# SYSTRAN/faster-whisper

Hardware: AMD Instinct MI355X
Metric: audio-sec/sec (RTF) large-v3 fp16 beam=5 batch=16 (higher is better)
Workload: dtype f16

## Files before the change

### faster_whisper_amd/_lib.py

```python
import ctypes as C
import os

import numpy as np

_HERE = os.path.dirname(os.path.abspath(__file__))
LIB_PATH = os.environ.get("FWAMD_LIB") or os.path.join(_HERE, "libfwamd.so")

FW_OK = 0
FW_EINVAL = -1
FW_ENODEV = -2
FW_ENOMEM = -3
FW_ERUNTIME = -4
FW_ENOSPC = -5

COMPUTE_FLOAT16 = 0
COMPUTE_INT8_FLOAT16 = 1
FW_DT_F32 = 0
FW_DT_F16 = 1
FW_MAX_ALIGN_HEADS = 64


class FwConfig(C.Structure):
    _fields_ = [
        ("n_mels", C.c_int32), ("n_audio_ctx", C.c_int32), ("d_model", C.c_int32), ("n_heads", C.c_int32),
        ("n_enc_layers", C.c_int32), ("n_dec_layers", C.c_int32), ("n_vocab", C.c_int32),
        ("n_text_ctx", C.c_int32), ("is_multilingual", C.c_int32),
        ("tok_eot", C.c_int32), ("tok_sot", C.c_int32), ("tok_lang_begin", C.c_int32), ("n_langs", C.c_int32),
        ("tok_translate", C.c_int32), ("tok_transcribe", C.c_int32), ("tok_sot_lm", C.c_int32),
        ("tok_sot_prev", C.c_int32), ("tok_no_speech", C.c_int32), ("tok_no_timestamps", C.c_int32),
        ("tok_timestamp_begin", C.c_int32),
        ("n_suppress_begin", C.c_int32), ("suppress_begin", C.c_int32 * 8),
        ("n_align_heads", C.c_int32), ("align_heads", C.c_int32 * (2 * FW_MAX_ALIGN_HEADS)),
    ]


class FwWeight(C.Structure):
    _fields_ = [("name", C.c_char_p), ("data", C.c_void_p), ("dtype", C.c_int32), ("ndim", C.c_int32),
                ("dims", C.c_int64 * 4)]


class FwGenOpts(C.Structure):
    _fields_ = [
        ("beam_size", C.c_int32), ("patience", C.c_float), ("num_hypotheses", C.c_int32),
        ("length_penalty", C.c_float), ("repetition_penalty", C.c_float), ("no_repeat_ngram_size", C.c_int32),
        ("max_length", C.c_int32), ("return_scores", C.c_int32), ("return_no_speech_prob", C.c_int32),
        ("max_initial_timestamp_index", C.c_int32), ("suppress_blank", C.c_int32),
        ("suppress_tokens", C.POINTER(C.c_int32)), ("n_suppress_tokens", C.c_int32),
        ("sampling_topk", C.c_int32), ("sampling_temperature", C.c_float), ("seed", C.c_uint64),
        ("min_new_tokens", C.c_int32),
    ]


class FwVadWeights(C.Structure):
    _fields_ = [
        ("stft_basis", C.c_void_p), ("conv_w", C.c_void_p * 4), ("conv_b", C.c_void_p * 4),
        ("lstm_w", C.c_void_p), ("lstm_r", C.c_void_p), ("lstm_b", C.c_void_p), ("dec_w", C.c_void_p),
        ("dec_b", C.c_float),
    ]


SYMBOLS = [
    "fw_last_error", "fw_abi_version", "fw_device_count",
    "fw_model_create", "fw_model_free", "fw_model_info", "fw_model_blob", "fw_model_create_from_blob_dev",
    "fw_model_set_decode_batch", "fw_model_decode_batch", "fw_model_join_decoder", "fw_model_decode_stats",
    "fw_model_set_merge_wait", "fw_model_set_decode_lanes", "fw_model_run_capacity", "fw_dec_big_min_rows", "fw_dec_big_min_rows_of", "fw_test_knob",
    "fw_test_idle_lead_chunks",
    "fw_pack_blob_size", "fw_pack_blob_copy", "fw_pack_blob_free",
    "fw_logmel", "fw_logmel_full",
    "fw_encode", "fw_encode_pcm", "fw_encode_pcm_dev", "fw_tensor_shape", "fw_tensor_to_host",
    "fw_tensor_from_host", "fw_tensor_free",
    "fw_generate", "fw_generate_lp", "fw_detect_language", "fw_align",
    "fw_prof_enable", "fw_prof_reset", "fw_prof_count", "fw_prof_name", "fw_prof_get", "fw_synchronize",
    "fw_dev_alloc", "fw_dev_free", "fw_dev_upload",
    "fw_test_gemm", "fw_test_layernorm", "fw_test_attention", "fw_test_dec_linear", "fw_test_dec_logits", "fw_test_logits_rules",
    "fw_test_dec_self_attn", "fw_test_dec_cross_attn", "fw_test_dec_cross_probs", "fw_test_dec_softmax_pick", "fw_bench_gemm", "fw_bench_dec_linear", "fw_bench_attention",
    "fw_bench_gemm_epi", "fw_bench_dec_linear_epi",
    "fw_test_gemm_ex", "fw_test_cross_kv_frag_index", "fw_test_quant_rows", "fw_test_layernorm_frag",
    "fw_test_dec_beam_update", "fw_test_dec_embed", "fw_test_align_post",
    "fw_test_logits_rules_lp", "fw_test_dec_beam_update_lp",
    "fw_test_logits_rules_smp_tab", "fw_test_graph_captures",
    "fw_vad_create", "fw_vad_forward", "fw_vad_free", "fw_vad_forward_dev", "fw_vad_forward_audio_dev",
    "fw_vad_forward_audio_batch_dev",
    "fw_flac_info", "fw_flac_decode",
    "fw_resample_filter", "fw_resample_dev", "fw_bench_resample",
]

_lib = None


class FwError(RuntimeError):
    pass


def load():
    global _lib
    if _lib is not None:
        return _lib
    if not os.path.exists(LIB_PATH):
        raise FwError(
            f"{LIB_PATH} not found: build it with `python -c 'import __graft_entry__ as g; g.build()'` "
            "(hipcc --offload-arch=gfx950). faster_whisper_amd has no CPU fallback.")
    lib = C.CDLL(LIB_PATH)
    vp, i32, i64, f32p = C.c_void_p, C.c_int32, C.c_int64, C.POINTER(C.c_float)
    i32p, i64p = C.POINTER(C.c_int32), C.POINTER(C.c_int64)
    lib.fw_last_error.restype = C.c_char_p
    lib.fw_abi_version.restype = i32
    lib.fw_device_count.restype = i32
    lib.fw_model_create.argtypes = [C.POINTER(FwConfig), C.POINTER(FwWeight), i32, i32, i32, i32, i32, C.POINTER(vp)]
    lib.fw_model_free.argtypes = [vp]
    lib.fw_model_free.restype = None
    lib.fw_model_info.argtypes = [vp, C.POINTER(FwConfig), i32p, i32p, i32p, i32p]
    lib.fw_model_blob.argtypes = [vp, C.POINTER(vp), i64p]
    lib.fw_model_create_from_blob_dev.argtypes = [C.POINTER(FwConfig), vp, i64, i32, i32, i32, i32, C.POINTER(vp)]
    lib.fw_model_set_decode_batch.argtypes = [vp, i32]
    lib.fw_model_decode_batch.argtypes = [vp]
    lib.fw_model_decode_batch.restype = i32
    lib.fw_model_run_capacity.argtypes = [vp]
    lib.fw_model_run_capacity.restype = i32
    lib.fw_dec_big_min_rows.restype = i32
    if hasattr(lib, "fw_dec_big_min_rows_of"):
        lib.fw_dec_big_min_rows_of.restype = i32
        lib.fw_dec_big_min_rows_of.argtypes = [i32, i32]
    if hasattr(lib, "fw_flac_info"):
        lib.fw_flac_info.argtypes = [vp, i64, i32p, i32p, i32p, i64p]
        lib.fw_flac_decode.argtypes = [vp, i64, vp, i64, i64p, i32p]
    if hasattr(lib, "fw_test_knob"):
        lib.fw_test_knob.argtypes = [i32, i32]
    if hasattr(lib, "fw_test_idle_lead_chunks"):
        lib.fw_test_idle_lead_chunks.argtypes = [i64, i32, i32, i64, i32]
        lib.fw_test_idle_lead_chunks.restype = i64
    lib.fw_model_join_decoder.argtypes = [vp, vp]
    lib.fw_model_set_merge_wait.argtypes = [vp, i32, i32]
    lib.fw_model_set_decode_lanes.argtypes = [vp, i32]
    lib.fw_model_decode_stats.argtypes = [vp, i64p, i64p, i64p, i32p]
    lib.fw_pack_blob_size.argtypes = [C.POINTER(FwConfig), C.POINTER(FwWeight), i32, i32, i64p, C.POINTER(vp)]
    lib.fw_pack_blob_copy.argtypes = [vp, vp, i64]
    lib.fw_pack_blob_free.argtypes = [vp]
    lib.fw_pack_blob_free.restype = None
    lib.fw_logmel.argtypes = [vp, vp, i64p, i32, vp, i32p]
    lib.fw_logmel_full.argtypes = [vp, vp, i64, vp, i64]
    lib.fw_encode.argtypes = [vp, vp, i32, C.POINTER(vp)]
    lib.fw_encode_pcm.argtypes = [vp, vp, i64p, i32, C.POINTER(vp)]
    lib.fw_encode_pcm_dev.argtypes = [vp, vp, i64p, i32, C.POINTER(vp)]
    lib.fw_tensor_shape.argtypes = [vp, i32p, i32p, i32p]
    lib.fw_tensor_to_host.argtypes = [vp, vp, vp]
    lib.fw_tensor_from_host.argtypes = [vp, vp, i32, C.POINTER(vp)]
    lib.fw_tensor_free.argtypes = [vp]
    lib.fw_tensor_free.restype = None
    lib.fw_generate.argtypes = [vp, vp, i32p, i32p, i32, C.POINTER(FwGenOpts), i32p, i32p, f32p, f32p]
    if hasattr(lib, "fw_generate_lp"):
        lib.fw_generate_lp.argtypes = [vp, vp, i32p, i32p, i32, C.POINTER(FwGenOpts), i32p, i32p, f32p, f32p, f32p, f32p]
    lib.fw_detect_language.argtypes = [vp, vp, i32, i32p, f32p]
    lib.fw_align.argtypes = [vp, vp, i32p, i32, i32p, i32p, i32p, i32, i32, i32, i32p, i32p, f32p]
    lib.fw_prof_enable.argtypes = [vp, i32]
    lib.fw_prof_enable.restype = None
    lib.fw_prof_reset.argtypes = [vp]
    lib.fw_prof_reset.restype = None
    lib.fw_prof_count.restype = i32
    lib.fw_prof_name.argtypes = [i32]
    lib.fw_prof_name.restype = C.c_char_p
    lib.fw_prof_get.argtypes = [vp, i32, C.POINTER(C.c_double), i64p, C.POINTER(C.c_double), C.POINTER(C.c_double)]
    lib.fw_synchronize.argtypes = [vp]
    lib.fw_dev_alloc.argtypes = [vp, i64, C.POINTER(vp)]
    lib.fw_dev_free.argtypes = [vp, vp]
    lib.fw_dev_upload.argtypes = [vp, vp, vp, i64]
    lib.fw_test_gemm.argtypes = [vp, vp, vp, vp, vp, i32, i32, i32, i32, i32, vp]
    lib.fw_test_dec_linear.argtypes = [vp, vp, vp, vp, vp, vp, vp, i32, i32, i32, i32, i32, vp, vp]
    lib.fw_test_dec_logits.argtypes = [vp, vp, i32, vp]
    lib.fw_test_logits_rules.argtypes = [vp, vp, i32, vp, i32, vp, C.POINTER(FwGenOpts), i32, vp, vp]
    if hasattr(lib, "fw_test_dec_self_attn"):
        lib.fw_test_dec_self_attn.argtypes = [vp, vp, vp, vp, vp, i32, i32, i32, i32, i32, i32, i32, i32, i32, i32, i32, vp]
        lib.fw_test_dec_cross_attn.argtypes = [vp, vp, vp, vp, i32, i32, i32, i32, i32, i32, vp, vp, i32, C.c_float, vp]
        lib.fw_test_dec_cross_probs.argtypes = [vp, vp, vp, i32, i32, i32, vp, i32, i32, i32, i32, vp]
        lib.fw_test_dec_softmax_pick.argtypes = [vp, vp, i32, i32, i32, vp, i32, vp]
    lib.fw_bench_attention.argtypes = [vp, i32, i32, i32, i32, i32, f32p]
    lib.fw_bench_gemm.argtypes = [vp, i32, i32, i32, i32, i32, i32, i32, i32, f32p]
    lib.fw_bench_dec_linear.argtypes = [vp, i32, i32, i32, i32, i32, i32, f32p]
    if hasattr(lib, "fw_bench_gemm_epi"):
        lib.fw_bench_gemm_epi.argtypes = [vp, i32, i32, i32, i32, i32, i32, i32, i32, i32, i32, i32, f32p]
        lib.fw_bench_dec_linear_epi.argtypes = [vp, i32, i32, i32, i32, i32, i32, i32, i32, i32, f32p]
    lib.fw_test_layernorm.argtypes = [vp, vp, vp, vp, i32, i32, vp]
    lib.fw_test_attention.argtypes = [vp, vp, vp, vp, i32, i32, i32, vp]
    if hasattr(lib, "fw_test_gemm_ex"):
        lib.fw_test_gemm_ex.argtypes = [vp, vp, i64, i64, i64, vp, vp, vp, i64, i64, i64, vp, i64, i64, i64, i64, i64,
                                        i32, i32, i32, i32, i32, i32, i32, i32, i32, vp, vp]
        lib.fw_test_cross_kv_frag_index.argtypes = [i32, i32, i32, vp]
        lib.fw_test_quant_rows.argtypes = [vp, vp, i32, i32, i64, vp, vp, i32, vp, vp]
        lib.fw_test_layernorm_frag.argtypes = [vp, vp, vp, vp, i32, i32, i32, vp]
    if hasattr(lib, "fw_test_dec_beam_update"):
        f32 = C.c_float
        lib.fw_test_dec_beam_update.argtypes = [vp, i32, i32, i32, i32, i32, i32, i32, i32, f32, i32, vp, vp, vp, vp, vp,
                                                i32, f32, vp, vp, vp, vp, vp, vp, vp, vp, vp, vp, vp]
        lib.fw_test_dec_embed.argtypes = [vp, vp, i32, vp, i32, vp, i32, i32, i32, i32, i32, i32, f32, vp, vp]
        lib.fw_test_align_post.argtypes = [vp, vp, i32, i32, i32, i32, vp, vp, i32, vp]
    if hasattr(lib, "fw_test_dec_beam_update_lp"):
        f32 = C.c_float
        lib.fw_test_logits_rules_lp.argtypes = [vp, vp, i32, vp, i32, vp, C.POINTER(FwGenOpts), i32, vp, vp, vp]
        lib.fw_test_dec_beam_update_lp.argtypes = [vp, i32, i32, i32, i32, i32, i32, i32, i32, f32, i32, vp, vp, vp, vp, vp,
                                                   vp, vp, i32, f32, vp, vp, vp, vp, vp, vp, vp, vp, vp, vp, vp, vp, vp]
    if hasattr(lib, "fw_test_graph_captures"):
        lib.fw_test_logits_rules_smp_tab.argtypes = [vp, vp, i32, vp, i32, vp, C.POINTER(FwGenOpts), i32, vp, vp, vp, vp, vp, vp]
        lib.fw_test_graph_captures.argtypes = [vp, i64p]
    lib.fw_vad_create.argtypes = [C.POINTER(FwVadWeights), C.POINTER(vp)]
    lib.fw_vad_forward.argtypes = [vp, vp, i64, i32, vp, vp, vp]
    lib.fw_vad_free.argtypes = [vp]
    lib.fw_vad_forward_dev.argtypes = [vp, i32, vp, i64, vp, vp, vp]
    if hasattr(lib, "fw_vad_forward_audio_dev"):
        lib.fw_vad_forward_audio_dev.argtypes = [vp, i32, vp, i64, vp, vp, vp]
    if hasattr(lib, "fw_vad_forward_audio_batch_dev"):
        lib.fw_vad_forward_audio_batch_dev.argtypes = [vp, i32, vp, vp, i32, vp, vp, vp]
    lib.fw_vad_free.restype = None
    if hasattr(lib, "fw_resample_dev"):
        f64 = C.c_double
        lib.fw_resample_filter.argtypes = [i32, i32, i32, f64, vp, i64p, i32p, i32p]
        lib.fw_resample_dev.argtypes = [i32, vp, i64, i32, i32, i32, f64, i32, vp, i64]
        lib.fw_bench_resample.argtypes = [i32, vp, i64, i32, i32, i32, f64, i32, i32, f32p]
    _lib = lib
    return lib


def check(rc: int):
    if rc == FW_OK:
        return
    msg = load().fw_last_error().decode("utf-8", "replace")
    if rc in (FW_EINVAL, FW_ENOSPC):
        raise ValueError(msg)
    raise RuntimeError(f"libfwamd error {rc}: {msg}")


def ptr(a: np.ndarray):
    return a.ctypes.data_as(C.c_void_p)


def as_i32p(a: np.ndarray):
    return a.ctypes.data_as(C.POINTER(C.c_int32))


def as_i64p(a: np.ndarray):
    return a.ctypes.data_as(C.POINTER(C.c_int64))


def as_f32p(a: np.ndarray):
    return a.ctypes.data_as(C.POINTER(C.c_float))
```

### faster_whisper_amd/csrc/attn_enc.hip

```cpp
#include "common.h"
#include "kernels.h"

#define AE_Q 128
#define AE_KV 64
#define AE_VSTRIDE 68
#define AE_LAG 5.0f

__global__ __launch_bounds__(256) void attn_enc_kernel(const half_t* __restrict__ q, const half_t* __restrict__ k,
                                                       int64_t ld, int64_t qk_bstride,
                                                       const half_t* __restrict__ vt, int64_t ldvt,
                                                       int64_t vt_bstride, half_t* __restrict__ out, int64_t ldo,
                                                       int64_t o_bstride, int T, int H, int n_pairs, int n_qt,
                                                       int order) {
  __shared__ __attribute__((aligned(16))) half_t sK[2][AE_KV * 64];
  __shared__ __attribute__((aligned(16))) half_t sV[2][64 * AE_VSTRIDE];

  const int tid = threadIdx.x, lane = tid & 63, wave = tid >> 6;
  const int hi = lane >> 5, l31 = lane & 31;
  const int xcd = blockIdx.x & 7, idx = blockIdx.x >> 3;
  const int pair = order ? (int)blockIdx.x / n_qt : (idx / n_qt) * 8 + xcd;
  if (pair >= n_pairs) return;
  const int b = pair / H, h = pair - b * H, q0 = (order ? (int)blockIdx.x % n_qt : idx % n_qt) * AE_Q;

  const half_t* qb = q + (size_t)b * qk_bstride + h * 64;
  const half_t* kb = k + (size_t)b * qk_bstride + h * 64;
  const half_t* vb = vt + (size_t)b * vt_bstride + (size_t)(h * 64) * ldvt;

  half8_t qf[4];
  {
    int qr = q0 + wave * 32 + l31;
    if (qr > T - 1) qr = T - 1;
    const half_t* qp = qb + (size_t)qr * ld + hi * 8;
#pragma unroll
    for (int ks = 0; ks < 4; ++ks) {
      half8_t v = *reinterpret_cast<const half8_t*>(qp + ks * 16);
#pragma unroll
      for (int e = 0; e < 8; ++e) v[e] = (half_t)((float)v[e] * (0.125f * 1.4426950408889634f));
      qf[ks] = v;
    }
  }

  const int c = tid & 7, r0 = tid >> 3;
  const int nkt = (T + AE_KV - 1) / AE_KV;
  intx4 rk[2], rv[2];
  auto gload = [&](int kt) {
#pragma unroll
    for (int i = 0; i < 2; ++i) {
      const int row = r0 + 32 * i;
      int key = kt * AE_KV + row;
      if (key > T - 1) key = T - 1;
      rk[i] = *reinterpret_cast<const intx4*>(kb + (size_t)key * ld + c * 8);
      rv[i] = *reinterpret_cast<const intx4*>(vb + (size_t)row * ldvt + kt * AE_KV + c * 8);
    }
  };
  auto lstore = [&](int buf) {
#pragma unroll
    for (int i = 0; i < 2; ++i) {
      const int row = r0 + 32 * i;
      *reinterpret_cast<intx4*>(&sK[buf][row * 64 + ((c ^ ((row >> 1) & 7)) << 3)]) = rk[i];
      intx2* dv = reinterpret_cast<intx2*>(&sV[buf][row * AE_VSTRIDE + c * 8]);
      dv[0] = intx2{rv[i][0], rv[i][1]};
      dv[1] = intx2{rv[i][2], rv[i][3]};
    }
  };

  gload(0);
  lstore(0);
  __syncthreads();

  floatx16 o[2] = {floatx16{0}, floatx16{0}};
  floatx16 lsum = floatx16{0};
  const half8_t ones8 = {(half_t)1.f, (half_t)1.f, (half_t)1.f, (half_t)1.f, (half_t)1.f, (half_t)1.f, (half_t)1.f, (half_t)1.f};
  float m_ref = 0.f;
  floatx16 cneg = floatx16{0};

  for (int kt = 0; kt < nkt; ++kt) {
    const int cur = kt & 1;
    const bool more = (kt + 1) < nkt;
    if (more) gload(kt + 1);

    floatx16 s[2];
#pragma unroll
    for (int ks = 0; ks < 4; ++ks) {
      const int chunk = ks * 2 + hi;
#pragma unroll
      for (int kb2 = 0; kb2 < 2; ++kb2) {
        const int row = kb2 * 32 + l31;
        const half8_t kf = *reinterpret_cast<const half8_t*>(&sK[cur][row * 64 + ((chunk ^ ((row >> 1) & 7)) << 3)]);
        s[kb2] = __builtin_amdgcn_mfma_f32_32x32x16_f16(kf, qf[ks], ks == 0 ? cneg : s[kb2], 0, 0, 0);
      }
    }
    const int kbase = kt * AE_KV + 4 * hi;
    const bool tail = (kt * AE_KV + AE_KV) > T;
    if (tail) {
#pragma unroll
      for (int kb2 = 0; kb2 < 2; ++kb2)
#pragma unroll
        for (int r = 0; r < 16; ++r) {
          const int key = kbase + kb2 * 32 + (r & 3) + 8 * (r >> 2);
          if (key >= T) s[kb2][r] = -1.0e30f;
        }
    }
    float mx = fmaxf(s[0][0], s[1][0]);
#pragma unroll
    for (int r = 1; r < 16; ++r) mx = __builtin_fmaxf(__builtin_fmaxf(mx, s[0][r]), s[1][r]);
    mx = pair32_max(mx);
    if (kt == 0 || __builtin_amdgcn_ballot_w64(mx > AE_LAG) != 0) {
      const float delta = kt == 0 ? mx : fmaxf(mx, 0.f);
      const float alpha = kt == 0 ? 1.f : __builtin_amdgcn_exp2f(-delta);
      m_ref += delta;
#pragma unroll
      for (int r = 0; r < 16; ++r) { cneg[r] = -m_ref; lsum[r] *= alpha; }
#pragma unroll
      for (int dt = 0; dt < 2; ++dt)
#pragma unroll
        for (int r = 0; r < 16; ++r) o[dt][r] *= alpha;
#pragma unroll
      for (int kb2 = 0; kb2 < 2; ++kb2)
#pragma unroll
        for (int r = 0; r < 16; ++r) s[kb2][r] -= delta;
    }
#pragma unroll
    for (int kb2 = 0; kb2 < 2; ++kb2)
#pragma unroll
      for (int r = 0; r < 16; ++r) s[kb2][r] = __builtin_amdgcn_exp2f(s[kb2][r]);

#pragma unroll
    for (int kb2 = 0; kb2 < 2; ++kb2)
#pragma unroll
      for (int ks2 = 0; ks2 < 2; ++ks2) {
        half8_t pf;
#pragma unroll
        for (int e = 0; e < 8; e += 2) {
          const half2_t h2 = {(half_t)s[kb2][ks2 * 8 + e], (half_t)s[kb2][ks2 * 8 + e + 1]};
          pf[e] = h2[0]; pf[e + 1] = h2[1];
        }
        lsum = __builtin_amdgcn_mfma_f32_32x32x16_f16(ones8, pf, lsum, 0, 0, 0);
        const int koff = kb2 * 32 + ks2 * 16 + 4 * hi;
#pragma unroll
        for (int dt = 0; dt < 2; ++dt) {
          const half_t* vr = &sV[cur][(dt * 32 + l31) * AE_VSTRIDE + koff];
          const half4_t v0 = *reinterpret_cast<const half4_t*>(vr);
          const half4_t v1 = *reinterpret_cast<const half4_t*>(vr + 8);
          half8_t vf;
#pragma unroll
          for (int e = 0; e < 4; ++e) { vf[e] = v0[e]; vf[4 + e] = v1[e]; }
          o[dt] = __builtin_amdgcn_mfma_f32_32x32x16_f16(vf, pf, o[dt], 0, 0, 0);
        }
      }

    if (more) lstore(cur ^ 1);
    __syncthreads();
  }

  const float inv = 1.0f / lsum[0];
  const int qr = q0 + wave * 32 + l31;
  if (qr < T) {
    half_t* op = out + (size_t)b * o_bstride + (size_t)qr * ldo + h * 64;
#pragma unroll
    for (int dt = 0; dt < 2; ++dt)
#pragma unroll
      for (int g = 0; g < 4; ++g) {
        half4_t ov;
#pragma unroll
        for (int e = 0; e < 4; ++e) ov[e] = (half_t)(o[dt][g * 4 + e] * inv);
        *reinterpret_cast<half4_t*>(op + dt * 32 + 8 * g + 4 * hi) = ov;
      }
  }
}

namespace fwk {
void launch_attn_enc(hipStream_t st, const half_t* q, const half_t* k, int64_t ld, int64_t qk_bstride,
                     const half_t* vt, int64_t ldvt, int64_t vt_bstride, half_t* out, int64_t ldo,
                     int64_t o_bstride, int B, int H, int T, int order) {
  const int n_qt = (T + AE_Q - 1) / AE_Q, n_pairs = B * H;
  const int grid = ((n_pairs + 7) / 8) * 8 * n_qt;
  attn_enc_kernel<<<grid, 256, 0, st>>>(q, k, ld, qk_bstride, vt, ldvt, vt_bstride, out, ldo, o_bstride, T, H, n_pairs, n_qt, order);
}
}
```

### faster_whisper_amd/csrc/hooks.hip

```cpp
#include "engine.h"

#include <math.h>
#include <string.h>

#include <algorithm>

#include "dec_kernels.h"
#include "kernels.h"

using namespace fw;
using fwd::FIN_CAP;
using fwd::GenDev;

namespace {

struct HookBufs {
  std::vector<void*> p;
  HookBufs() = default;
  HookBufs(const HookBufs&) = delete;
  HookBufs& operator=(const HookBufs&) = delete;
  ~HookBufs() { for (void* q : p) (void)hipFree(q); }
  template <typename T>
  int alloc(T** dst, size_t n) {
    int rc = dev_alloc_t(dst, n);
// ... 432 lines not shown
  Model* m = &fm->impl;
  std::lock_guard<std::mutex> lk(m->mu);
  FW_HIP(hipSetDevice(m->device));
  hipStream_t st = m->stream;
  const size_t wn = (size_t)N * K;
  const int copies = (int)std::max<size_t>(2, ((size_t)640 << 20) / (wn * 2));
  const size_t rp = ((size_t)R + 15) / 16 * 16, on = rp * N;
  const int ocopies = (int)std::max<size_t>(2, ((size_t)640 << 20) / (on * 2));
  HookBufs db;
  half_t *dW, *dX, *dO, *dF, *dB;
  float *dS, *dC;
  std::vector<uint16_t> stage;
  int rc;
  if ((rc = db.alloc(&dW, wn * copies)) || (rc = db.alloc(&dX, rp * K)) || (rc = db.alloc(&dO, on * ocopies)) ||
      (rc = db.alloc(&dF, on)) || (rc = db.alloc(&dB, (size_t)N)) || (rc = db.alloc(&dS, (size_t)N)) || (rc = db.alloc(&dC, (size_t)N)) ||
      (rc = fill_lcg(dW, wn, stage, 2463534242u, 1e-3f)) || (rc = fill_lcg(dX, rp * K, stage, 2463534242u, 1e-3f)) ||
      (rc = db.zero(dO, on * ocopies * 2, st)) || (rc = db.zero(dB, (size_t)N * 2, st)) || (rc = db.zero(dS, (size_t)N * 4, st)) ||
      (rc = db.zero(dC, (size_t)N * 4, st)))
    return rc;
  for (int c = 1; c < copies; ++c) FW_HIP(hipMemcpy(dW + (size_t)c * wn, dW, wn * 2, hipMemcpyDeviceToDevice));
  float ms = 0.f;
  rc = time_launches(st, 4, iters, [&](int i) {
    const half_t* w = dW + (size_t)(i % copies) * wn;
    half_t* o = dO + (size_t)(i % ocopies) * on;
    half_t* op = (outs & 1) ? o : nullptr;
    half_t* of = (outs & 2) ? dF : nullptr;
    const half_t* r = res ? o : nullptr;
    const half_t* b = lnf ? nullptr : dB;
    const float *s1 = lnf ? dS : nullptr, *cf = lnf ? dC : nullptr;
    if (variant >= 10) return fwd::launch_dec_gemm_big(st, variant - 10, dX, w, b, s1, cf, r, N, op, N, of, R, N, K, act);
    if (variant == 5) return fwd::launch_dec_gemm_skinny(st, dX, w, b, s1, cf, r, N, op, N, of, R, N, K, act);
    return fwd::launch_dec_gemm_frag(st, dX, w, b, s1, cf, r, N, op, N, of, R, N, K, act);
  }, &ms);
  if (rc == LAUNCH_REFUSED) { set_error("fw_bench_dec_linear_epi: unsupported shape / variant"); return FW_EINVAL; }
  if (rc) return rc;
  *us_out = ms * 1000.f / (float)iters;
  return FW_OK;
}

int32_t fw_test_layernorm(fw_model* fm, const float* x, const float* g, const float* b, int32_t rows, int32_t d,
                          float* out) {
  return test_layernorm_impl(fm, x, g, b, rows, d, 0, out);
}
int32_t fw_test_layernorm_frag(fw_model* fm, const float* x, const float* g, const float* b, int32_t rows, int32_t d,
                               int32_t frag, float* out) {
  return test_layernorm_impl(fm, x, g, b, rows, d, frag, out);
}

int32_t fw_test_quant_rows(fw_model* fm, const float* x, int32_t rows, int32_t d, int64_t ldx, const float* ln_g,
                           const float* ln_b, int32_t frag, int8_t* xq, float* scale) {
  FW_CHECK_ARG(fm && x && xq && scale && rows >= 1 && rows <= (1 << 20), "bad argument");
  FW_CHECK_ARG((ln_g == nullptr) == (ln_b == nullptr), "ln_g and ln_b go together");
  FW_CHECK_ARG(d >= 64 && d % 64 == 0 && d <= (ln_g ? 1536 : 5120), "d %% 64 == 0, d <= 1536 with LayerNorm, <= 5120 without");
  FW_CHECK_ARG(ldx >= d && ldx % 8 == 0 && ldx <= (1 << 20), "ldx >= d, ldx %% 8 == 0");
  Model* m = &fm->impl;
  std::lock_guard<std::mutex> lk(m->mu);
  FW_HIP(hipSetDevice(m->device));
  const int R16 = (rows + 15) / 16 * 16;
  std::vector<int8_t> hq((size_t)R16 * d);
  HookBufs db;
  half_t *dx, *dg = nullptr, *dlb = nullptr;
  int8_t* dq;
  float* ds;
  int rc;
  if ((rc = db.upload_f16(&dx, x, (size_t)(rows - 1) * ldx + d)) || (ln_g && (rc = db.upload_f16(&dg, ln_g, d))) ||
      (ln_b && (rc = db.upload_f16(&dlb, ln_b, d))) || (rc = db.alloc(&dq, hq.size())) || (rc = db.alloc(&ds, (size_t)R16)) ||
      (rc = db.zero(dq, hq.size(), m->stream)))
    return rc;
  fwk::launch_quant_rows(m->stream, dx, ldx, dg, dlb, dq, ds, rows, d, frag ? 1 : 0);
  FW_HIP(hipStreamSynchronize(m->stream));
  if ((rc = download(hq.data(), dq, hq.size())) || (rc = download(scale, ds, (size_t)rows))) return rc;
  for (int r = 0; r < rows; ++r)
    for (int k = 0; k < d; ++k) xq[(size_t)r * d + k] = hq[frag ? frag_pos(r, k, d, 64) : (size_t)r * d + k];
  return FW_OK;
}

int32_t fw_test_cross_kv_frag_index(int32_t vt, int32_t kvp, int32_t N, int64_t* idx) {
  FW_CHECK_ARG(idx && kvp >= 32 && kvp % 32 == 0 && N >= 64 && N % 64 == 0, "need kvp %% 32 == 0, N %% 64 == 0");
  for (int mm = 0; mm < kvp; ++mm)
    for (int n = 0; n < N; ++n) idx[(size_t)mm * N + n] = (int64_t)cross_kv_frag_pos(vt != 0, kvp, mm, n);
  return FW_OK;
}

int32_t fw_test_gemm_ex(fw_model* fm, const float* A, int64_t a_elems, int64_t lda, int64_t a_bstride, const float* W,
                        const float* bias, const float* res, int64_t r_elems, int64_t ldr, int64_t r_bstride, float* C,
                        int64_t c_elems, int64_t c_off, int64_t ldc, int64_t c_bstride, int64_t c_lstride, int32_t M,
                        int32_t N, int32_t K, int32_t batch, int32_t n_layers, int32_t act, int32_t trans,
                        int32_t head_rows, int32_t use_int8, const float* ln_g, const float* ln_b) {
  FW_CHECK_ARG(fm && A && W && C, "null argument");
  const int64_t dim_max = 1 << 20, cnt_max = 1 << 12, str_max = (int64_t)1 << 40;
  FW_CHECK_ARG(M >= 1 && N >= 1 && K >= 1 && M <= dim_max && N <= dim_max && K <= dim_max, "bad M / N / K");
  FW_CHECK_ARG(batch >= 1 && n_layers >= 1 && batch <= cnt_max && n_layers <= cnt_max, "bad batch / n_layers");
  for (int64_t v : {a_elems, lda, a_bstride, r_elems, ldr, r_bstride, c_elems, c_off, ldc, c_bstride, c_lstride})
    FW_CHECK_ARG(v >= 0 && v <= str_max, "negative or oversized count / stride");
  FW_CHECK_ARG(act == 0 || act == 1, "act is 0 or 1");
  FW_CHECK_ARG((ln_g == nullptr) == (ln_b == nullptr) && (!ln_g || use_int8), "ln_g / ln_b: both, and only with use_int8");
  const bool rowmajor = !trans && head_rows == 0;
  FW_CHECK_ARG(!res || (rowmajor && n_layers == 1), "a residual needs the row-major single-layer form");
  FW_CHECK_ARG(n_layers == 1 || (!use_int8 && act == 0), "the layered launch is fp16 without activation");
  FW_CHECK_ARG(head_rows == 0 || (head_rows > 0 && head_rows % 32 == 0 && head_rows >= M && N % 64 == 0),
               "fragment-major output: head_rows %% 32 == 0, head_rows >= M, N %% 64 == 0");
  FW_CHECK_ARG(c_off % 8 == 0 && c_lstride % 8 == 0, "c_off and c_lstride must be multiples of 8");
  if (use_int8) FW_CHECK_ARG(lda == K && a_bstride == (int64_t)M * K, "int8: A is contiguous [batch * M][K]");
  const int64_t a_last = (int64_t)(batch - 1) * a_bstride + (int64_t)(M - 1) * lda + (K - 1);
  FW_CHECK_ARG(a_last < a_elems, "the launch reads A[%lld], a_elems = %lld", (long long)a_last, (long long)a_elems);
  if (res) {
    const int64_t r_last = (int64_t)(batch - 1) * r_bstride + (int64_t)(M - 1) * ldr + (N - 1);
    FW_CHECK_ARG(r_last < r_elems, "the launch reads res[%lld], r_elems = %lld", (long long)r_last, (long long)r_elems);
  }
  const int64_t chunk_last = head_rows > 0 ? (int64_t)(N / 64 - 1) * head_rows * 64 + (int64_t)((M - 1) / 32 + 1) * 2048 - 1
                             : trans       ? (int64_t)(N - 1) * ldc + (M - 1)
                                           : (int64_t)(M - 1) * ldc + (N - 1);
  const int64_t c_last = c_off + (int64_t)(n_layers - 1) * c_lstride + (int64_t)(batch - 1) * c_bstride + chunk_last;
  FW_CHECK_ARG(c_last < c_elems, "the launch writes C[%lld], c_elems = %lld", (long long)c_last, (long long)c_elems);

  Model* m = &fm->impl;
  std::lock_guard<std::mutex> lk(m->mu);
  if (use_int8) {
    const int64_t T = m->cfg.n_audio_ctx;
    if (m->compute_type != FW_COMPUTE_INT8_FLOAT16 || (int64_t)batch * M * K > (int64_t)m->max_batch * T * 4 * m->cfg.d_model ||
        (int64_t)batch * M > (int64_t)m->max_batch * T || (ln_g && K > 1536)) {
      set_error("int8 gemm test needs an int8_float16 model, batch*M*K within its quantisation workspace, K <= 1536 with LayerNorm");
      return FW_EINVAL;
    }
  }
  FW_HIP(hipSetDevice(m->device));
  HookBufs db;
  half_t *dA, *dW, *dB = nullptr, *dR = nullptr, *dC, *dG = nullptr, *dLb = nullptr;
  int rc;
  if ((rc = db.upload_f16(&dA, A, (size_t)a_elems)) || (rc = db.upload_f16(&dW, W, (size_t)n_layers * N * K)) ||
      (bias && (rc = db.upload_f16(&dB, bias, (size_t)n_layers * N))) || (res && (rc = db.upload_f16(&dR, res, (size_t)r_elems))) ||
      (rc = db.upload_f16(&dC, C, (size_t)c_elems)) ||
      (ln_g && ((rc = db.upload_f16(&dG, ln_g, K)) || (rc = db.upload_f16(&dLb, ln_b, K)))))
    return rc;
  LinearW L{dW, dB, nullptr, nullptr, nullptr, nullptr, N, K};
  if (use_int8) {
    int8_t* dWq;
    float* dWs;
    if ((rc = upload_quant_w(db, W, N, K, [&](int n, int k) { return (size_t)n * K + k; }, &dWq, &dWs))) return rc;
    L.wq = dWq; L.wscale = dWs;
    LNW ln{dG, dLb};
    rc = run_linear_i8(m, L, dA, ln_g ? &ln : nullptr, dC + c_off, ldc, c_bstride, dR, ldr, r_bstride, M, batch, act,
                       trans != 0, head_rows);
  } else if (n_layers > 1) {
    rc = run_linear_layers(m, L, n_layers, (int64_t)N * K, bias ? N : 0, dA, lda, a_bstride, dC + c_off, ldc, c_bstride,
                           c_lstride, M, batch, trans != 0, head_rows, nullptr);
  } else {
    rc = run_linear(m, L, dA, lda, a_bstride, dC + c_off, ldc, c_bstride, dR, ldr, r_bstride, M, batch, act, trans != 0,
                    head_rows, nullptr);
  }
  return rc ? rc : download_f16(m->stream, C, dC, (size_t)c_elems);
}

int32_t fw_test_attention(fw_model* fm, const float* q, const float* k, const float* v, int32_t B, int32_t H,
                          int32_t T, float* out) {
  FW_CHECK_ARG(fm && q && k && v && out, "null argument");
  Model* m = &fm->impl;
  std::lock_guard<std::mutex> lk(m->mu);
  FW_HIP(hipSetDevice(m->device));
  const int d = H * 64, tp = (T + 63) / 64 * 64;
  const size_t n = (size_t)B * T * d;
  std::vector<float> vt((size_t)B * d * tp, 0.f);
  for (int b = 0; b < B; ++b)
    for (int t = 0; t < T; ++t)
      for (int c = 0; c < d; ++c) vt[((size_t)b * d + c) * tp + t] = v[((size_t)b * T + t) * d + c];
  HookBufs db;
  half_t *dq, *dk, *dvt, *dout;
  int rc;
  if ((rc = db.upload_f16(&dq, q, n)) || (rc = db.upload_f16(&dk, k, n)) || (rc = db.upload_f16(&dvt, vt.data(), vt.size())) ||
      (rc = db.alloc(&dout, n)))
    return rc;
  fwk::launch_attn_enc(m->stream, dq, dk, d, (int64_t)T * d, dvt, tp, (int64_t)d * tp, dout, d, (int64_t)T * d, B, H,
                       T);
  return download_f16(m->stream, out, dout, n);
}

int32_t fw_bench_attention(fw_model* fm, int32_t B, int32_t H, int32_t T, int32_t variant, int32_t iters, float* ms_out) {
  FW_CHECK_ARG(fm && ms_out && B > 0 && H > 0 && T > 0 && iters > 0, "bad argument");
  Model* m = &fm->impl;
  std::lock_guard<std::mutex> lk(m->mu);
  FW_HIP(hipSetDevice(m->device));
  const int d = H * 64, tp = (T + 63) / 64 * 64;
  const size_t nqk = (size_t)B * T * 2 * d, nvt = (size_t)B * d * tp, no = (size_t)B * T * d;
  HookBufs db;
  half_t *dqk, *dvt, *dout;
  std::vector<uint16_t> stage;
  int rc;
  if ((rc = db.alloc(&dqk, nqk)) || (rc = db.alloc(&dvt, nvt)) || (rc = db.alloc(&dout, no)) ||
      (rc = fill_lcg(dqk, nqk, stage, 777u, 2e-3f)) || (rc = fill_lcg(dvt, nvt, stage, 777u, 2e-3f)))
    return rc;
  float ms = 0.f;
  rc = time_launches(m->stream, 1, iters, [&](int) {
    fwk::launch_attn_enc(m->stream, dqk, dqk + d, 2 * d, (int64_t)T * 2 * d, dvt, tp, (int64_t)d * tp, dout, d, (int64_t)T * d, B,
                         H, T, variant);
    return 0;
  }, &ms);
  if (rc) return rc;
  *ms_out = ms / (float)iters;
  return FW_OK;
}

int32_t fw_test_dec_self_attn(fw_model* fm, const float* qkv, float* kcache, float* vcache, const uint8_t* kvidx,
                              int32_t n_chunks, int32_t kmul, int32_t Kbeam, int32_t H, int32_t n_ctx, int32_t cache_ctx,
                              int32_t pos_fixed, int32_t P, int32_t step, int32_t blk_n, int32_t frag, float* out) {
  FW_CHECK_ARG(fm && qkv && kcache && vcache && kvidx && out, "null argument");
  FW_CHECK_ARG(n_chunks >= 1 && H >= 1 && kmul >= 1 && kmul <= 16 && Kbeam >= 1 && Kbeam <= 255, "bad geometry");
  FW_CHECK_ARG(n_ctx >= 1 && n_ctx <= 448 && cache_ctx >= 1 && cache_ctx <= n_ctx, "need 1 <= cache_ctx <= n_ctx <= 448");
  FW_CHECK_ARG(blk_n >= 0 && (blk_n == 0 ? kmul <= Kbeam : (kmul == blk_n && pos_fixed >= 0)),
               "blk_n = 0: kmul <= Kbeam; blk_n > 0: kmul == blk_n and pos_fixed >= 0");
  const int pos0 = pos_fixed >= 0 ? pos_fixed : P - 1 + step;
  const int pos_last = pos0 + (blk_n > 0 ? blk_n - 1 : 0);
  FW_CHECK_ARG(pos0 >= 0 && pos_last < cache_ctx, "positions %d..%d outside the cache (%d)", pos0, pos_last, cache_ctx);
  const int d = H * 64, R = n_chunks * kmul, R16 = (R + 15) / 16 * 16, R_total = n_chunks * Kbeam;
  FW_CHECK_ARG(blk_n == 0 || fwd::self_attn_block_ok(n_ctx, cache_ctx, d, R_total), "position blocks need n_ctx %% 4 == 0");
  const size_t n_tab = (size_t)2 * R_total * n_ctx, n_cache = (size_t)R_total * H * cache_ctx * 64;
  for (size_t i = 0; i < n_tab; ++i)
    FW_CHECK_ARG(kvidx[i] < Kbeam, "kvidx[%zu] = %d is not a beam of %d", i, (int)kvidx[i], Kbeam);
  Model* m = &fm->impl;
  std::lock_guard<std::mutex> lk(m->mu);
  FW_HIP(hipSetDevice(m->device));
  hipStream_t st = m->stream;
  HookBufs db;
  half_t *d_qkv, *d_kc, *d_vc, *d_out;
  uint8_t* d_idx;
  int* d_step;
  int rc;
  if ((rc = db.upload_f16(&d_qkv, qkv, (size_t)R * 3 * d)) || (rc = db.upload_f16(&d_kc, kcache, n_cache)) ||
      (rc = db.upload_f16(&d_vc, vcache, n_cache)) || (rc = db.alloc(&d_out, (size_t)R16 * d)) ||
      (rc = db.upload(&d_idx, kvidx, n_tab)) || (rc = db.upload(&d_step, &step, 1)) ||
      (rc = db.zero(d_out, (size_t)R16 * d * 2, st)))
    return rc;
  fwd::launch_self_attn(st, d_qkv, d, d_kc, d_vc, n_ctx, cache_ctx, H, d_idx, Kbeam, kmul, d_out, R, d_step, pos_fixed, P,
                        R_total, frag ? 1 : 0, blk_n);
  FW_HIP(hipGetLastError());
  if ((rc = download_f16(st, kcache, d_kc, n_cache)) || (rc = download_f16(st, vcache, d_vc, n_cache))) return rc;
  return frag ? download_f16_frag(st, out, d_out, R, d) : download_f16(st, out, d_out, (size_t)R * d);
}

int32_t fw_test_dec_cross_attn(fw_model* fm, const float* q, const float* k, const float* v, int32_t n_enc, int32_t T,
                               int32_t H, int32_t B, int32_t kmul, int32_t kv_div, const int32_t* slot_map,
                               const int32_t* done, int32_t frag, float k_pad, float* out) {
  FW_CHECK_ARG(fm && q && k && v && slot_map && out, "null argument");
  FW_CHECK_ARG(n_enc >= 1 && T >= 1 && H >= 1 && B >= 1 && kmul >= 1 && kmul <= 16 && kv_div >= 1, "bad geometry");
  const int n_map = (B + kv_div - 1) / kv_div;
  for (int i = 0; i < n_map; ++i)
    FW_CHECK_ARG(slot_map[i] >= 0 && slot_map[i] < n_enc, "slot_map[%d] = %d outside [0, %d)", i, slot_map[i], n_enc);
  const int d = H * 64, kvp = (T + 31) / 32 * 32, R = B * kmul, R16 = (R + 15) / 16 * 16;
  const size_t blk = (size_t)d * kvp;
  std::vector<float> kf((size_t)n_enc * blk), vf((size_t)n_enc * blk, 0.f);
  for (int e = 0; e < n_enc; ++e)
    for (int t = 0; t < kvp; ++t)
      for (int n = 0; n < d; ++n) {
        const size_t src = ((size_t)e * T + t) * d + n;
        kf[e * blk + cross_kv_frag_pos(false, kvp, t, n)] = t < T ? k[src] : k_pad;
        if (t < T) vf[e * blk + cross_kv_frag_pos(true, kvp, t, n)] = v[src];
      }
  std::vector<float> of((size_t)R16 * d, 0.f);
  for (int r = 0; r < R; ++r)
    for (int n = 0; n < d; ++n) of[frag ? frag_pos(r, n, d, 32) : (size_t)r * d + n] = out[(size_t)r * d + n];
  Model* m = &fm->impl;
  std::lock_guard<std::mutex> lk(m->mu);
  FW_HIP(hipSetDevice(m->device));
  HookBufs db;
  half_t *d_q, *d_k, *d_vt, *d_out;
  int *d_map, *d_done = nullptr;
  int rc;
  if ((rc = db.upload_f16(&d_q, q, (size_t)R * d)) || (rc = db.upload_f16(&d_k, kf.data(), kf.size())) ||
      (rc = db.upload_f16(&d_vt, vf.data(), vf.size())) || (rc = db.upload_f16(&d_out, of.data(), of.size())) ||
      (rc = db.upload(&d_map, slot_map, (size_t)n_map)) || (done && (rc = db.upload(&d_done, done, (size_t)B))))
    return rc;
  fwd::launch_cross_attn(m->stream, d_q, d, d_k, d_vt, T, kvp, kmul, d_out, B, H, d_done, kv_div, frag ? 1 : 0, d_map);
  FW_HIP(hipGetLastError());
  return frag ? download_f16_frag(m->stream, out, d_out, R, d) : download_f16(m->stream, out, d_out, (size_t)R * d);
}

int32_t fw_test_dec_cross_probs(fw_model* fm, const float* q, const float* k, int32_t B, int32_t T, int32_t H,
                                const int32_t* heads, int32_t n_sel, int32_t n_tok, int32_t tok_idx, int32_t blk_n,
                                float* probs) {
  FW_CHECK_ARG(fm && q && k && heads && probs, "null argument");
  const int blk = blk_n > 0 ? blk_n : 1;
  FW_CHECK_ARG(B >= 1 && T >= 1 && H >= 1 && n_sel >= 1 && blk_n >= 0 && blk <= 16, "bad geometry");
  FW_CHECK_ARG(tok_idx >= 0 && tok_idx + blk <= n_tok, "tokens %d..%d outside [0, %d)", tok_idx, tok_idx + blk - 1, n_tok);
  for (int i = 0; i < n_sel; ++i) FW_CHECK_ARG(heads[i] >= 0 && heads[i] < H, "heads[%d] = %d outside [0, %d)", i, heads[i], H);
  const int d = H * 64, kvp = (T + 31) / 32 * 32;
  const size_t blkk = (size_t)d * kvp, n_probs = (size_t)B * n_sel * n_tok * T;
  std::vector<float> kf((size_t)B * blkk, 0.f);
  for (int b = 0; b < B; ++b)
    for (int t = 0; t < T; ++t)
      for (int n = 0; n < d; ++n) kf[b * blkk + cross_kv_frag_pos(false, kvp, t, n)] = k[((size_t)b * T + t) * d + n];
  Model* m = &fm->impl;
  std::lock_guard<std::mutex> lk(m->mu);
  FW_HIP(hipSetDevice(m->device));
  HookBufs db;
  half_t *d_q, *d_k;
  int* d_heads;
  float* d_p;
  int rc;
  if ((rc = db.upload_f16(&d_q, q, (size_t)B * blk * d)) || (rc = db.upload_f16(&d_k, kf.data(), kf.size())) ||
      (rc = db.upload(&d_heads, heads, (size_t)n_sel)) || (rc = db.upload(&d_p, probs, n_probs)))
    return rc;
  fwd::launch_cross_probs(m->stream, d_q, d, d_k, T, kvp, d_heads, n_sel, n_sel, d_p, n_tok, tok_idx, B, blk_n);
  FW_HIP(hipGetLastError());
  FW_HIP(hipStreamSynchronize(m->stream));
  return download(probs, d_p, n_probs);
}

int32_t fw_test_dec_softmax_pick(fw_model* fm, const float* logits, int32_t rows, int32_t V, int32_t row_mul,
                                 const int32_t* target, int32_t nospeech, float* out) {
  FW_CHECK_ARG(fm && logits && target && out, "null argument");
  FW_CHECK_ARG(rows >= 1 && V >= 1 && row_mul >= 1, "bad geometry");
  FW_CHECK_ARG(!nospeech || (target[0] >= 0 && target[0] < V), "no-speech id %d outside [0, %d)", target[0], V);
  Model* m = &fm->impl;
  std::lock_guard<std::mutex> lk(m->mu);
  FW_HIP(hipSetDevice(m->device));
  HookBufs db;
  const size_t n_lg = (size_t)rows * row_mul * V;
  float *d_lg, *d_out;
  int* d_t;
  int rc;
  if ((rc = db.upload(&d_lg, logits, n_lg)) || (rc = db.alloc(&d_out, (size_t)rows)) || (rc = db.alloc(&d_t, (size_t)rows))) return rc;
  FW_HIP(hipMemcpy(d_t, target, (size_t)(nospeech ? 1 : rows) * sizeof(int), hipMemcpyHostToDevice));
  if (nospeech) fwd::launch_nospeech(m->stream, d_lg, V, row_mul, target[0], d_out, rows);
  else fwd::launch_token_prob(m->stream, d_lg, V, d_t, d_out, 1, 0, rows, row_mul);
  FW_HIP(hipGetLastError());
  FW_HIP(hipStreamSynchronize(m->stream));
  return download(out, d_out, (size_t)rows);
}
// ... 288 lines not shown
```

### profiles/attn_bench.py

```python
import ctypes as C
import os
import sys

sys.path.insert(0, os.path.dirname(os.path.dirname(os.path.abspath(__file__))))
from faster_whisper_amd import Whisper, _lib, get_config, synthetic_weights


def main():
    cfg = get_config("micro")
    m = Whisper("synthetic:micro", device="cuda", files={"config": cfg, "weights": synthetic_weights(cfg, seed=1)},
                max_batch_size=1, max_beam_size=1)
    h = m._replicas[0].handle
    ms = C.c_float()
    B, H, T = 16, 20, 1500
    fl = 4.0 * B * H * T * T * 64
    only = int(sys.argv[1]) if len(sys.argv) > 1 else -1
    for rnd in range(3):
        for variant, what in ((0, "XCD-aware grid"), (1, "round-3 grid")):
            if only >= 0 and variant != only:
                continue
            _lib.check(m._lib.fw_bench_attention(h, B, H, T, variant, 50, C.byref(ms)))
            print(f"round {rnd} {what}: {ms.value * 1e3:.1f} us per launch, {fl / ms.value / 1e9:.0f} TFLOP/s", flush=True)


if __name__ == "__main__":
    main()
```

Measured before the change: 3181.

## Stage encoder attention K/V tiles via global_load_lds DMA instead of registers

Adds a templated DMA path to the encoder flash-attention kernel that loads K and V tiles straight from global memory into LDS with global_load_lds. This replaces the register-staged gload/lstore double buffer and uses one waitcnt+barrier per tile. The V tile gets an XOR-swizzled 128-byte row layout, and the running-max subtraction is folded into a per-tile MFMA accumulator init. The DMA path becomes the default, with the old register path kept behind order bit 2. The intent is to cut register pressure and VGPR-to-LDS store instructions on the critical path, at the risk of new LDS bank conflicts or extra barrier stalls.

```diff
diff --git a/faster_whisper_amd/_lib.py b/faster_whisper_amd/_lib.py
--- a/faster_whisper_amd/_lib.py
+++ b/faster_whisper_amd/_lib.py
@@ -72,7 +72,7 @@
     "fw_generate", "fw_generate_lp", "fw_detect_language", "fw_align",
     "fw_prof_enable", "fw_prof_reset", "fw_prof_count", "fw_prof_name", "fw_prof_get", "fw_synchronize",
     "fw_dev_alloc", "fw_dev_free", "fw_dev_upload",
-    "fw_test_gemm", "fw_test_layernorm", "fw_test_attention", "fw_test_dec_linear", "fw_test_dec_logits", "fw_test_logits_rules",
+    "fw_test_gemm", "fw_test_layernorm", "fw_test_attention", "fw_test_attention_form", "fw_test_dec_linear", "fw_test_dec_logits", "fw_test_logits_rules",
     "fw_test_dec_self_attn", "fw_test_dec_cross_attn", "fw_test_dec_cross_probs", "fw_test_dec_softmax_pick", "fw_bench_gemm", "fw_bench_dec_linear", "fw_bench_attention",
     "fw_bench_gemm_epi", "fw_bench_dec_linear_epi",
     "fw_test_gemm_ex", "fw_test_cross_kv_frag_index", "fw_test_quant_rows", "fw_test_layernorm_frag",
@@ -181,6 +181,8 @@
         lib.fw_bench_dec_linear_epi.argtypes = [vp, i32, i32, i32, i32, i32, i32, i32, i32, i32, f32p]
     lib.fw_test_layernorm.argtypes = [vp, vp, vp, vp, i32, i32, vp]
     lib.fw_test_attention.argtypes = [vp, vp, vp, vp, i32, i32, i32, vp]
+    if hasattr(lib, "fw_test_attention_form"):
+        lib.fw_test_attention_form.argtypes = [vp, vp, vp, vp, i32, i32, i32, i32, vp]
     if hasattr(lib, "fw_test_gemm_ex"):
         lib.fw_test_gemm_ex.argtypes = [vp, vp, i64, i64, i64, vp, vp, vp, i64, i64, i64, vp, i64, i64, i64, i64, i64,
                                         i32, i32, i32, i32, i32, i32, i32, i32, i32, vp, vp]
diff --git a/faster_whisper_amd/csrc/attn_enc.hip b/faster_whisper_amd/csrc/attn_enc.hip
--- a/faster_whisper_amd/csrc/attn_enc.hip
+++ b/faster_whisper_amd/csrc/attn_enc.hip
@@ -1,21 +1,33 @@
 #include "common.h"
 #include "kernels.h"
+#include <type_traits>
 
 #define AE_Q 128
 #define AE_KV 64
 #define AE_VSTRIDE 68
 #define AE_LAG 5.0f
-
+#define AE_TILE_BYTES (AE_KV * 128)
+#define AE_BUF_BYTES (2 * AE_TILE_BYTES)
+
+#define AE_DMA_BARRIER()                                        \
+  do {                                                          \
+    asm volatile("s_waitcnt vmcnt(0) lgkmcnt(0)" ::: "memory"); \
+    __builtin_amdgcn_s_barrier();                               \
+    asm volatile("" ::: "memory");                              \
+  } while (0)
+
+template <bool DMA>
 __global__ __launch_bounds__(256) void attn_enc_kernel(const half_t* __restrict__ q, const half_t* __restrict__ k,
                                                        int64_t ld, int64_t qk_bstride,
                                                        const half_t* __restrict__ vt, int64_t ldvt,
                                                        int64_t vt_bstride, half_t* __restrict__ out, int64_t ldo,
                                                        int64_t o_bstride, int T, int H, int n_pairs, int n_qt,
                                                        int order) {
-  __shared__ __attribute__((aligned(16))) half_t sK[2][AE_KV * 64];
-  __shared__ __attribute__((aligned(16))) half_t sV[2][64 * AE_VSTRIDE];
-
-  const int tid = threadIdx.x, lane = tid & 63, wave = tid >> 6;
+  constexpr int V_BASE = 2 * AE_TILE_BYTES;
+  constexpr int V_BYTES = 64 * AE_VSTRIDE * 2;
+  __shared__ __attribute__((aligned(16))) char smem[DMA ? 2 * AE_BUF_BYTES : V_BASE + 2 * V_BYTES];
+
+  const int tid = threadIdx.x, lane = tid & 63, wave = __builtin_amdgcn_readfirstlane(tid >> 6);
   const int hi = lane >> 5, l31 = lane & 31;
   const int xcd = blockIdx.x & 7, idx = blockIdx.x >> 3;
   const int pair = order ? (int)blockIdx.x / n_qt : (idx / n_qt) * 8 + xcd;
@@ -40,8 +52,9 @@
     }
   }
 
+  const int nkt = (T + AE_KV - 1) / AE_KV;
+
   const int c = tid & 7, r0 = tid >> 3;
-  const int nkt = (T + AE_KV - 1) / AE_KV;
   intx4 rk[2], rv[2];
   auto gload = [&](int kt) {
 #pragma unroll
@@ -54,19 +67,45 @@
     }
   };
   auto lstore = [&](int buf) {
+    half_t* sKb = reinterpret_cast<half_t*>(smem + buf * AE_TILE_BYTES);
+    half_t* sVb = reinterpret_cast<half_t*>(smem + V_BASE + buf * V_BYTES);
 #pragma unroll
     for (int i = 0; i < 2; ++i) {
       const int row = r0 + 32 * i;
-      *reinterpret_cast<intx4*>(&sK[buf][row * 64 + ((c ^ ((row >> 1) & 7)) << 3)]) = rk[i];
-      intx2* dv = reinterpret_cast<intx2*>(&sV[buf][row * AE_VSTRIDE + c * 8]);
+      *reinterpret_cast<intx4*>(&sKb[row * 64 + ((c ^ ((row >> 1) & 7)) << 3)]) = rk[i];
+      intx2* dv = reinterpret_cast<intx2*>(&sVb[row * AE_VSTRIDE + c * 8]);
       dv[0] = intx2{rv[i][0], rv[i][1]};
       dv[1] = intx2{rv[i][2], rv[i][3]};
     }
   };
 
-  gload(0);
-  lstore(0);
-  __syncthreads();
+  const int drow = wave * 8 + (lane >> 3);
+  const unsigned dchunk = (unsigned)(((lane & 7) ^ ((drow >> 1) & 7)) * 16);
+  const unsigned ldb = (unsigned)ld * 2u;
+  const unsigned dvoff = (unsigned)drow * (unsigned)ldvt * 2u + dchunk;
+  auto issue = [&](int kt, int buf) {
+    char* dst = smem + buf * AE_BUF_BYTES + wave * 1024;
+#pragma unroll
+    for (int i = 0; i < 2; ++i) {
+      int key = kt * AE_KV + drow + 32 * i;
+      if (key > T - 1) key = T - 1;
+      const unsigned ko = (unsigned)key * ldb + dchunk;
+      const unsigned vo = dvoff + (unsigned)(32 * i) * (unsigned)ldvt * 2u + (unsigned)kt * (AE_KV * 2u);
+      __builtin_amdgcn_global_load_lds((const __attribute__((address_space(1))) void*)(reinterpret_cast<const char*>(kb) + (size_t)ko),
+                                       (__attribute__((address_space(3))) void*)(dst + i * 4096), 16, 0, 0);
+      __builtin_amdgcn_global_load_lds((const __attribute__((address_space(1))) void*)(reinterpret_cast<const char*>(vb) + (size_t)vo),
+                                       (__attribute__((address_space(3))) void*)(dst + AE_TILE_BYTES + i * 4096), 16, 0, 0);
+    }
+  };
+  const int fkey = (l31 >> 1) & 7;
+
+  if (DMA) {
+    issue(0, 0);
+  } else {
+    gload(0);
+    lstore(0);
+    __syncthreads();
+  }
 
   floatx16 o[2] = {floatx16{0}, floatx16{0}};
   floatx16 lsum = floatx16{0};
@@ -74,20 +113,33 @@
   float m_ref = 0.f;
   floatx16 cneg = floatx16{0};
 
-  for (int kt = 0; kt < nkt; ++kt) {
-    const int cur = kt & 1;
+  auto tile = [&](int kt, auto CUR) {
+    const int cur = CUR;
     const bool more = (kt + 1) < nkt;
-    if (more) gload(kt + 1);
+    if (DMA) {
+      AE_DMA_BARRIER();
+      if (more) issue(kt + 1, cur ^ 1);
+    } else {
+      if (more) gload(kt + 1);
+    }
+    const char* sKc = smem + (DMA ? cur * AE_BUF_BYTES : cur * AE_TILE_BYTES);
+    const char* sVc = smem + (DMA ? cur * AE_BUF_BYTES + AE_TILE_BYTES : V_BASE + cur * V_BYTES);
 
     floatx16 s[2];
+    floatx16 cref;
+    {
+      const float nm = -m_ref;
+#pragma unroll
+      for (int r = 0; r < 16; ++r) cref[r] = nm;
+    }
 #pragma unroll
     for (int ks = 0; ks < 4; ++ks) {
       const int chunk = ks * 2 + hi;
 #pragma unroll
       for (int kb2 = 0; kb2 < 2; ++kb2) {
         const int row = kb2 * 32 + l31;
-        const half8_t kf = *reinterpret_cast<const half8_t*>(&sK[cur][row * 64 + ((chunk ^ ((row >> 1) & 7)) << 3)]);
-        s[kb2] = __builtin_amdgcn_mfma_f32_32x32x16_f16(kf, qf[ks], ks == 0 ? cneg : s[kb2], 0, 0, 0);
+        const half8_t kf = *reinterpret_cast<const half8_t*>(sKc + row * 128 + ((chunk ^ fkey) << 4));
+        s[kb2] = __builtin_amdgcn_mfma_f32_32x32x16_f16(kf, qf[ks], ks == 0 ? (DMA ? cref : cneg) : s[kb2], 0, 0, 0);
       }
     }
     const int kbase = kt * AE_KV + 4 * hi;
@@ -110,7 +162,7 @@
       const float alpha = kt == 0 ? 1.f : __builtin_amdgcn_exp2f(-delta);
       m_ref += delta;
 #pragma unroll
-      for (int r = 0; r < 16; ++r) { cneg[r] = -m_ref; lsum[r] *= alpha; }
+      for (int r = 0; r < 16; ++r) { if (!DMA) cneg[r] = -m_ref; lsum[r] *= alpha; }
 #pragma unroll
       for (int dt = 0; dt < 2; ++dt)
 #pragma unroll
@@ -137,11 +189,21 @@
         }
         lsum = __builtin_amdgcn_mfma_f32_32x32x16_f16(ones8, pf, lsum, 0, 0, 0);
         const int koff = kb2 * 32 + ks2 * 16 + 4 * hi;
+        const int ch = kb2 * 4 + ks2 * 2;
 #pragma unroll
         for (int dt = 0; dt < 2; ++dt) {
-          const half_t* vr = &sV[cur][(dt * 32 + l31) * AE_VSTRIDE + koff];
-          const half4_t v0 = *reinterpret_cast<const half4_t*>(vr);
-          const half4_t v1 = *reinterpret_cast<const half4_t*>(vr + 8);
+          const char* vrow = sVc + (dt * 32 + l31) * (DMA ? 128 : AE_VSTRIDE * 2);
+          const char* p0 = DMA ? vrow + ((ch ^ fkey) << 4) + 8 * hi : vrow + koff * 2;
+          const char* p1 = DMA ? vrow + (((ch + 1) ^ fkey) << 4) + 8 * hi : vrow + koff * 2 + 16;
+          half4_t v0, v1;
+          if (DMA) {
+            typedef const volatile __attribute__((address_space(3))) half4_t* lds_v4;
+            v0 = *(lds_v4)(p0);
+            v1 = *(lds_v4)(p1);
+          } else {
+            v0 = *reinterpret_cast<const half4_t*>(p0);
+            v1 = *reinterpret_cast<const half4_t*>(p1);
+          }
           half8_t vf;
 #pragma unroll
           for (int e = 0; e < 4; ++e) { vf[e] = v0[e]; vf[4 + e] = v1[e]; }
@@ -149,9 +211,13 @@
         }
       }
 
-    if (more) lstore(cur ^ 1);
-    __syncthreads();
-  }
+    if (!DMA) {
+      if (more) lstore(cur ^ 1);
+      __syncthreads();
+    }
+  };
+
+  for (int kt = 0; kt < nkt; ++kt) tile(kt, kt & 1);
 
   const float inv = 1.0f / lsum[0];
   const int qr = q0 + wave * 32 + l31;
@@ -175,6 +241,9 @@
                      int64_t o_bstride, int B, int H, int T, int order) {
   const int n_qt = (T + AE_Q - 1) / AE_Q, n_pairs = B * H;
   const int grid = ((n_pairs + 7) / 8) * 8 * n_qt;
-  attn_enc_kernel<<<grid, 256, 0, st>>>(q, k, ld, qk_bstride, vt, ldvt, vt_bstride, out, ldo, o_bstride, T, H, n_pairs, n_qt, order);
+  if (order & 2)
+    attn_enc_kernel<false><<<grid, 256, 0, st>>>(q, k, ld, qk_bstride, vt, ldvt, vt_bstride, out, ldo, o_bstride, T, H, n_pairs, n_qt, order & 1);
+  else
+    attn_enc_kernel<true><<<grid, 256, 0, st>>>(q, k, ld, qk_bstride, vt, ldvt, vt_bstride, out, ldo, o_bstride, T, H, n_pairs, n_qt, order & 1);
 }
 }
diff --git a/faster_whisper_amd/csrc/hooks.hip b/faster_whisper_amd/csrc/hooks.hip
--- a/faster_whisper_amd/csrc/hooks.hip
+++ b/faster_whisper_amd/csrc/hooks.hip
@@ -608,9 +608,10 @@
   return rc ? rc : download_f16(m->stream, C, dC, (size_t)c_elems);
 }
 
-int32_t fw_test_attention(fw_model* fm, const float* q, const float* k, const float* v, int32_t B, int32_t H,
-                          int32_t T, float* out) {
+int32_t fw_test_attention_form(fw_model* fm, const float* q, const float* k, const float* v, int32_t B, int32_t H,
+                               int32_t T, int32_t variant, float* out) {
   FW_CHECK_ARG(fm && q && k && v && out, "null argument");
+  FW_CHECK_ARG(B > 0 && H > 0 && T > 0 && variant >= 0 && variant <= 3, "bad geometry or variant");
   Model* m = &fm->impl;
   std::lock_guard<std::mutex> lk(m->mu);
   FW_HIP(hipSetDevice(m->device));
@@ -627,8 +628,13 @@
       (rc = db.alloc(&dout, n)))
     return rc;
   fwk::launch_attn_enc(m->stream, dq, dk, d, (int64_t)T * d, dvt, tp, (int64_t)d * tp, dout, d, (int64_t)T * d, B, H,
-                       T);
+                       T, variant);
   return download_f16(m->stream, out, dout, n);
+}
+
+int32_t fw_test_attention(fw_model* fm, const float* q, const float* k, const float* v, int32_t B, int32_t H,
+                          int32_t T, float* out) {
+  return fw_test_attention_form(fm, q, k, v, B, H, T, 0, out);
 }
 
 int32_t fw_bench_attention(fw_model* fm, int32_t B, int32_t H, int32_t T, int32_t variant, int32_t iters, float* ms_out) {
diff --git a/profiles/attn_bench.py b/profiles/attn_bench.py
--- a/profiles/attn_bench.py
+++ b/profiles/attn_bench.py
@@ -16,7 +16,8 @@
     fl = 4.0 * B * H * T * T * 64
     only = int(sys.argv[1]) if len(sys.argv) > 1 else -1
     for rnd in range(3):
-        for variant, what in ((0, "XCD-aware grid"), (1, "round-3 grid")):
+        for variant, what in ((0, "LDS-DMA staging, XCD-aware grid"), (2, "register staging, XCD-aware grid"),
+                              (1, "LDS-DMA staging, round-3 grid")):
             if only >= 0 and variant != only:
                 continue
             _lib.check(m._lib.fw_bench_attention(h, B, H, T, variant, 50, C.byref(ms)))
```

Result: no change. 3178, median of 2 (-0.1%).
